# lazzati-astro/MCRaT

Hardware: AMD Instinct MI355X
Metric: photon-scatter-events/sec at 1e6 photons, 2D FLASH jet (higher is better)
Workload: dtype f64

## Files before the change

### include/mcrat_hip.h

```cpp
#ifndef MCRAT_HIP_H
#define MCRAT_HIP_H

#include <stddef.h>
#include <stdint.h>

#ifdef __cplusplus
extern "C" {
#endif
#if defined(__GNUC__)
#pragma GCC visibility push(default)
#endif

#define MCRAT_HIP_ABI_VERSION 1

#define MCRAT_HIP_OK        0
#define MCRAT_HIP_EINVAL   (-1)
#define MCRAT_HIP_ENODEV   (-2)
#define MCRAT_HIP_ENOMEM   (-3)
#define MCRAT_HIP_EHIP     (-4)
#define MCRAT_HIP_ESTATE   (-5)
#define MCRAT_HIP_EREFUSED (-6)

#define MCRAT_HIP_CARTESIAN        0
#define MCRAT_HIP_SPHERICAL        1
// ... 169 lines not shown
                            const mcrat_hip_outflow *outflow, mcrat_hip_ingest_result *result);

typedef struct mcrat_hip_hydro_columns {
    int num_elements;
    double *r0, *r1, *r2, *r0_size, *r1_size, *r2_size;
    double *v0, *v1, *v2;
    double *dens, *dens_lab, *pres, *temp, *gamma;
    double *r, *theta;
} mcrat_hip_hydro_columns;
int mcrat_hip_get_hydro(mcrat_hip_ctx *ctx, mcrat_hip_hydro_columns *out);

typedef struct mcrat_hip_output_columns {
    int count;
    double *p0, *p1, *p2, *p3;
    double *comv_p0, *comv_p1, *comv_p2, *comv_p3;
    double *r0, *r1, *r2;
    double *s0, *s1, *s2, *s3;
    double *num_scatt, *weight;
    char   *type;
} mcrat_hip_output_columns;
int mcrat_hip_get_output(mcrat_hip_ctx *ctx, mcrat_hip_output_columns *out);
int mcrat_hip_convert_comptonized(mcrat_hip_ctx *ctx, int *num_converted);
int mcrat_hip_get_photons_range(mcrat_hip_ctx *ctx, int first, int count, mcrat_hip_photon *records);

typedef struct mcrat_hip_outbox mcrat_hip_outbox;
int  mcrat_hip_outbox_create(mcrat_hip_ctx *ctx, mcrat_hip_outbox **box);
void mcrat_hip_outbox_destroy(mcrat_hip_outbox *box);
int  mcrat_hip_outbox_post(mcrat_hip_ctx *ctx, mcrat_hip_outbox *box, int want_records, int want_output);
int  mcrat_hip_outbox_wait(mcrat_hip_outbox *box, const mcrat_hip_photon **records, int *n_records, mcrat_hip_output_columns *cols);

typedef struct mcrat_hip_cyclosynch {
    int    b_field_calc;
    double epsilon_b;
    double rebin_e_perc, rebin_ang, rebin_ang_phi;
    int    scatt_frame_number, inj_frame_number;
} mcrat_hip_cyclosynch;
int mcrat_hip_set_hydro_extras(mcrat_hip_ctx *ctx, const double *dens, const double *B0, const double *B1, const double *B2);
int mcrat_hip_emit_cyclosynch_pool(mcrat_hip_ctx *ctx, const mcrat_hip_cyclosynch *cs, double r_inj, double ph_weight, int maximum_photons,
                                   double theta_min, double theta_max, double fps, uint64_t seed, int *num_emitted, double *ph_weight_adjusted,
                                   int *integrals_not_converged);
int mcrat_hip_rebin_cyclosynch(mcrat_hip_ctx *ctx, const mcrat_hip_cyclosynch *cs, int max_photons, int *empty_bins, int *num_cyclosynch_ph_emit,
                               int *scatt_cyclosynch_num_ph);
typedef struct mcrat_hip_cyclosynch_counts {
    int    num_cyclosynch_ph_emit, scatt_cyclosynch_num_ph, frame_abs_cnt;
    int    rebins;
    int    integrals_not_converged;
// ... 249 lines not shown
```

### mcrat_amd/csrc/device_types.hpp

```cpp
#pragma once
#include <stddef.h>
#include <stdint.h>

namespace mcrat {

constexpr double A_RAD = 7.56e-15;
constexpr double C_LIGHT = 2.99792458e10;
constexpr double PL_CONST = 6.6260755e-27;
constexpr double K_B = 1.380658e-16;
constexpr double M_P = 1.6726231e-24;
constexpr double THOM_X_SECT = 6.65246e-25;
constexpr double M_EL = 9.1093879e-28;

constexpr int GEOM_CARTESIAN = 0, GEOM_SPHERICAL = 1, GEOM_CYLINDRICAL = 2, GEOM_POLAR = 3;
constexpr int DIM_TWO = 0, DIM_TWO_POINT_FIVE = 1, DIM_THREE = 2;

constexpr unsigned FLAG_RECALC = 1u;
constexpr unsigned FLAG_MOVES = 2u;
constexpr unsigned FLAG_VALID = 4u;
constexpr unsigned FLAG_TAU_FRESH = 8u;

constexpr int TOPK = 4;
constexpr int MAX_SEG = 8;
constexpr int STEP_BLOCK = 256;
constexpr int STEP_QCAP = 1024;
#ifndef MCRAT_EVENT_BLOCK
#define MCRAT_EVENT_BLOCK 256
#endif
constexpr int SHORTLIST_CAP = MCRAT_EVENT_BLOCK;
constexpr int EVENT_BLOCK = MCRAT_EVENT_BLOCK;

struct PhotonDev {
    double *r0, *r1, *r2;
    double *p0, *p1, *p2, *p3;
    double *c0, *c1, *c2, *c3;
    double *s0, *s1, *s2, *s3;
    double *num_scatt;
    double *weight;
    double *tau;
    double *tts;
    double *u0, *u1, *u2;
    double *ntau;
    double *tau_next;
// ... 189 lines not shown
```

### mcrat_amd/csrc/engine.hip

```cpp
#include <hip/hip_runtime.h>
#include <algorithm>
#include <chrono>
#include <cmath>
#include <cstdio>
#include <cstdlib>
#include <cstring>
#include <mutex>
#include <new>
#include <string>
#include <vector>

#include "../../include/mcrat_hip.h"
#include "device_types.hpp"
#include "launch.hpp"
#include "observe_plan.hpp"
#include "sky_plan.hpp"
#include "sightline_plan.hpp"
#include "radfield_plan.hpp"
#include "comoving_plan.hpp"
#include "photon_cols.hpp"
#include "photon_plan.hpp"
#include "rng.hpp"

using namespace mcrat;
// ... 1734 lines not shown
    HIPCHK(c, hipMemcpyAsync(l->photons, c->aos_buf, bytes, hipMemcpyDeviceToHost, c->stream));
    HIPCHK(c, hipStreamSynchronize(c->stream));
    if (c->cfg.cyclosynchrotron_switch) {
        int nulls = 0;
        for (int i = 0; i < n; ++i) nulls += l->photons[i].type == 'N';
        l->num_null_photons = nulls;
        l->num_photons = n - nulls;
    }
    return MCRAT_HIP_OK;
}

extern "C" int mcrat_hip_get_photons_range(mcrat_hip_ctx *c, int first, int count, mcrat_hip_photon *records)
{
    if (!c || !records || first < 0 || count <= 0) return MCRAT_HIP_EINVAL;
    if (!c->have_photons) return MCRAT_HIP_ESTATE;
    if ((long long)first + count > c->ph.n) return MCRAT_HIP_EINVAL;
    int rc = flush_pending(c);
    if (rc) return rc;
    const size_t bytes = sizeof(mcrat_hip_photon) * (size_t)count;
    if ((rc = ensure_aos(c, bytes))) return rc;
    HIPCHK(c, hipMemsetAsync(c->aos_buf, 0, bytes, c->stream));
    HIPCHK(c, launch_soa_to_aos(c->ph, c->aos_buf, first, count, c->stream));
    HIPCHK(c, hipMemcpyAsync(records, c->aos_buf, bytes, hipMemcpyDeviceToHost, c->stream));
    HIPCHK(c, hipStreamSynchronize(c->stream));
    return MCRAT_HIP_OK;
}

extern "C" int mcrat_hip_convert_comptonized(mcrat_hip_ctx *c, int *num_converted)
{
    if (!c) return MCRAT_HIP_EINVAL;
    if (!c->have_photons) return MCRAT_HIP_ESTATE;
    int rc = ensure_aos(c, sizeof(unsigned));
    if (rc) return rc;
    unsigned n = 0;
    HIPCHK(c, hipMemsetAsync(c->aos_buf, 0, sizeof(unsigned), c->stream));
    HIPCHK(c, launch_convert_comptonized(c->ph, static_cast<unsigned *>(c->aos_buf), c->stream));
    HIPCHK(c, hipMemcpyAsync(&n, c->aos_buf, sizeof n, hipMemcpyDeviceToHost, c->stream));
    HIPCHK(c, hipStreamSynchronize(c->stream));
    if (num_converted) *num_converted = (int)n;
    return MCRAT_HIP_OK;
}

static size_t output_scan_ints(long long nblk) { return (size_t)nblk + 1 + grid_scan_scratch_ints(nblk); }
static int write_output(mcrat_hip_ctx *c, const OutputLayout &lay, void *base, long long nblk, unsigned long long total, OutputCols *oc)
{
    char *b = static_cast<char *>(base);
// ... 2505 lines not shown
```

### mcrat_amd/csrc/kernels.hip

```cpp
#include <hip/hip_runtime.h>
#include <limits.h>
#include <math.h>
#include <stdio.h>
#include <type_traits>
#include "device_types.hpp"
#include "launch.hpp"
#include "sc_exchange.hpp"
#include "physics.hpp"
#include "photon_cols.hpp"
#include "rng.hpp"
#include "cs_device.hpp"

#if !defined(MCRAT_TAU_TABLE_TU) || !defined(MCRAT_TU_DIMS)
#error "compile kernels.hip through kernels_d*.hip / kernels_table_d*.hip"
#endif
#define MCRAT_NS_CAT2(a, b) a##b
#define MCRAT_NS_CAT(a, b) MCRAT_NS_CAT2(a, b)
#if MCRAT_TAU_TABLE_TU
#define MCRAT_TU_NS MCRAT_NS_CAT(tau_table_d, MCRAT_TU_DIMS)
#else
#define MCRAT_TU_NS MCRAT_NS_CAT(tau_direct_d, MCRAT_TU_DIMS)
#endif

namespace mcrat {
// ... 204 lines not shown
        }
        if (queue == 1) bucket = phys::grid_bucket_of<DIMS>(hy.grid, a0, a1, a2);
        if (queue) return INFINITY;
        if (MC_DIAG(DIAG_SKIP_SAMPLE)) return 1e-3 + (double)i * 1e-12 + (double)(bits & 1) * 0.0 + ntau * 0.0;
        return sample_free_time(ntau, bits);
    }
    if (cell != -1) ph.idx(i) = -1;
    return 1e12 / C_LIGHT;
}

__device__ __forceinline__ double free_time_from_log(double ntau, double log_u) { return div_by_c(ntau * log_u); }

struct TableSite {
    uint64_t seed, pass;
    uint32_t stream, slot_base;
    int first;
    int mode;
    bool deferred;
    double norm, eps, theta;
    __device__ __forceinline__ TableSite(const RngKey &key, unsigned long long iter, int first_ = 0, int mode_ = 0)
        : seed(key.seed), pass(iter), stream(key.stream), slot_base(key.slot_base), first(first_), mode(mode_), deferred(false), norm(1), eps(0), theta(0) {}
};

template <int DIMS, int GEOM, bool LOGS = false, class PH>
__device__ __forceinline__ double slow_one(const PH &ph, const HydroDev &hy, int i, bool relocate, int bucket, bool count_it,
                                           uint64_t bits, int &relocated, int &not_found, TableSite &ts)
{
    const double r0 = ph.r0(i), r1 = ph.r1(i), r2 = ph.r2(i);
    const double p0 = ph.p0(i), p1 = ph.p1(i), p2 = ph.p2(i), p3 = ph.p3(i);
    const unsigned fl = ph.flags(i);
    int cell;
    bool need_tau = (fl & FLAG_RECALC) != 0;
    bool new_cell = false;
    double fa = 0, fb = 0, fc = 0, fw = 0, fnsig = 0, fgam = 1, fkf = 0.5;
    double a0 = 0, a1 = 0, a2 = 0;
    if (MC_DIAG(DIAG_SLOW_EMPTY)) { ph.tts(i) = 1e-3 + i * 1e-12; return 1e-3 + i * 1e-12; }
    if (MC_DIAG(DIAG_SLOW_NO_SEARCH)) relocate = false;
    if (relocate) {
        phys::hydro_coords<DIMS, GEOM>(r0, r1, r2, a0, a1, a2);
        FatCell hit;
        cell = phys::find_in_bucket<DIMS>(hy, bucket, a0, a1, a2, hit);
        ph.idx(i) = cell;
        if (cell != -1) {
            fa = hit.a; fb = hit.b; fc = hit.c; fw = hit.w; fnsig = hit.nsig; fgam = hit.gam; fkf = phys::kf_of_gamma(hit.gam);
            new_cell = true;
            need_tau = true;
            if (count_it) relocated += 1;
        } else {
            not_found += 1;
        }
    } else {
        cell = ph.idx(i);
        if (cell != -1) {
            const CellFluid f = hy.fluid[cell];
            fa = f.a; fb = f.b; fc = f.c; fw = f.w; fnsig = f.nsig;
        }
    }
    double t;
    if (MC_DIAG(DIAG_SLOW_NO_PHYSICS)) need_tau = false;
    if (cell != -1) {
        double ntau;
        if (need_tau) {
            double cphi, sphi;
            if (new_cell) phys::relocation_azimuth<DIMS, GEOM>(r0, r1, a0, cphi, sphi);
            else phys::cos_sin_of_atan2(r1, r0, cphi, sphi);
            double beta[3];
            phys::beta_from_record<DIMS>(fa, fb, fc, cphi, sphi, beta);
            double comv0 = 0;
            if (new_cell) {
                const double lab[4] = {p0, p1, p2, p3};
                double comv[4];
                phys::boost_with<true>(beta, fgam, fkf, lab, comv);
                ph.c0(i) = comv[0]; ph.c1(i) = comv[1]; ph.c2(i) = comv[2]; ph.c3(i) = comv[3];
                comv0 = comv[0];
            }
            double norm = 1.0;
            if constexpr (TABLE_MODE) {
                if (!new_cell) comv0 = ph.c0(i);
                if (ts.mode == 2) {
                    norm = ts.norm;
                } else if (phys::thermal_cross_section_lookup(hy, comv0, hy.temp[cell], norm, ts.eps, ts.theta)) {
                    if (ts.mode == 1) {
                        ts.deferred = true;
                        if (new_cell && count_it) relocated -= 1;
                        return 0.0;
                    }
                    norm = phys::table_fallback_lane(ts.eps, ts.theta, ts.seed, ts.pass, ts.slot_base + (uint32_t)(i - ts.first), ts.stream, hy.hot_fallback_calls);
                    atomicAdd(hy.table_fallbacks, 1);
                }
            }
            const double tau = phys::optical_depth_staged(beta, fw, fnsig, p1, p2, p3, norm);
            ntau = -phys::rcp_nr(tau);
            ph.tau(i) = tau;
            ph.ntau(i) = ntau;
            if (fl & FLAG_RECALC) ph.flags(i) = (unsigned char)(fl & ~(FLAG_RECALC | FLAG_TAU_FRESH));
        } else {
            ntau = ph.ntau(i);
        }
        t = LOGS ? free_time_from_log(ntau, __longlong_as_double((long long)bits)) : sample_free_time(ntau, bits);
    } else {
        t = 1e12 / C_LIGHT;
    }
    ph.tts(i) = t;
    return t;
}

struct LockstepProbe {
    const int *cached;
    bool force;
    bool *same;
};

template <int DIMS, int GEOM, int K, bool LOGS, bool COVERED, class PH>
__device__ __forceinline__ void relocate_lockstep_impl(const PH &ph, const HydroDev &hy, const int (&slot)[K], bool (&todo)[K],
                                                       const double (&r0)[K], const double (&r1)[K], const double (&a0)[K], const double (&a1)[K],
                                                       const double (&a2)[K], const int (&code)[K], const uint64_t (&bits)[K], const unsigned (&fl)[K],
                                                       bool count_it, double (&t)[K], int &relocated, const LockstepProbe *probe)
{
    static_assert(!TABLE_MODE, "DIRECT optical depths");
    const GridDev &g = hy.grid;
    double p0[K], p1[K], p2[K], p3[K];
    bool take[K];
    FatCell f[K];
    if constexpr (COVERED) {
        int cell[K];
#pragma unroll
        for (int k = 0; k < K; ++k) {
            take[k] = todo[k] && code[k] >= 0 && (code[k] & GRID_CODE_HINT_OK) != 0;
            cell[k] = phys::covered_cell<DIMS>(g, take[k] ? code[k] : 0);
            const int i = slot[k];
            p0[k] = ph.p0(i); p1[k] = ph.p1(i); p2[k] = ph.p2(i); p3[k] = ph.p3(i);
        }
#pragma unroll
        for (int k = 0; k < K; ++k) {
            take[k] = take[k] & (cell[k] >= 0);
            phys::fat_from_fluid(hy.fluid, take[k] ? cell[k] : 0, f[k]);
// ... 2 lines not shown
        BucketDir d[K];
#pragma unroll
        for (int k = 0; k < K; ++k) {
            take[k] = todo[k] && code[k] >= 0;
            d[k] = g.dir[take[k] ? (code[k] & GRID_CODE_BUCKET_MASK) : 0];
            const int i = slot[k];
            p0[k] = ph.p0(i); p1[k] = ph.p1(i); p2[k] = ph.p2(i); p3[k] = ph.p3(i);
        }
#pragma unroll
        for (int k = 0; k < K; ++k) {
            const unsigned hint = (d[k].hints >> (4 * ((code[k] >> GRID_CODE_OCT_SHIFT) & 7))) & 15u;
            take[k] = take[k] & (d[k].n > 0) & ((code[k] & GRID_CODE_HINT_OK) != 0) & (hint != GRID_NO_HINT);
            f[k] = g.cells[take[k] ? d[k].e0 + (int)hint : 0];
        }
    }
    double comv[K][4], tau[K], ntau[K];
#pragma unroll
    for (int k = 0; k < K; ++k) {
        if constexpr (!COVERED) take[k] = take[k] & phys::well_in_fat_cell<DIMS>(f[k], a0[k], a1[k], a2[k]);
        double cphi, sphi;
        phys::relocation_azimuth<DIMS, GEOM>(r0[k], r1[k], a0[k], cphi, sphi);
        double beta[3];
        phys::beta_from_record<DIMS>(f[k].a, f[k].b, f[k].c, cphi, sphi, beta);
        const double lab[4] = {p0[k], p1[k], p2[k], p3[k]};
        phys::boost_with<true>(beta, f[k].gam, phys::kf_of_gamma(f[k].gam), lab, comv[k]);
        tau[k] = phys::optical_depth_staged(beta, f[k].w, f[k].nsig, p1[k], p2[k], p3[k], 1.0);
        ntau[k] = -phys::rcp_nr(tau[k]);
        t[k] = LOGS ? free_time_from_log(ntau[k], __longlong_as_double((long long)bits[k])) : sample_free_time(ntau[k], bits[k]);
    }
#pragma unroll
    for (int k = 0; k < K; ++k)
        asm volatile("" : "+v"(comv[k][0]), "+v"(comv[k][1]), "+v"(comv[k][2]), "+v"(comv[k][3]), "+v"(tau[k]), "+v"(ntau[k]), "+v"(t[k]));
#pragma unroll
    for (int k = 0; k < K; ++k) {
        if (!take[k]) continue;
        if (probe) {
            probe->same[k] = !probe->force && f[k].cell == probe->cached[k];
            if (probe->same[k]) { todo[k] = false; continue; }
        }
        const int i = slot[k];
        ph.idx(i) = f[k].cell;
        ph.c0(i) = comv[k][0]; ph.c1(i) = comv[k][1]; ph.c2(i) = comv[k][2]; ph.c3(i) = comv[k][3];
        ph.tau(i) = tau[k];
        ph.ntau(i) = ntau[k];
        if (fl[k] & FLAG_RECALC) ph.flags(i) = (unsigned char)(fl[k] & ~(FLAG_RECALC | FLAG_TAU_FRESH));
        ph.tts(i) = t[k];
        if (count_it) relocated += 1;
        todo[k] = false;
    }
}
template <int DIMS, int GEOM, int K, bool LOGS = false, class PH>
__device__ __forceinline__ void relocate_lockstep(const PH &ph, const HydroDev &hy, const int (&slot)[K], bool (&todo)[K],
                                                  const double (&r0)[K], const double (&r1)[K], const double (&a0)[K], const double (&a1)[K],
                                                  const double (&a2)[K], const int (&code)[K], const uint64_t (&bits)[K], const unsigned (&fl)[K],
                                                  bool count_it, double (&t)[K], int &relocated, const LockstepProbe *probe = nullptr)
{
    if (hy.grid.cov_back) relocate_lockstep_impl<DIMS, GEOM, K, LOGS, true>(ph, hy, slot, todo, r0, r1, a0, a1, a2, code, bits, fl, count_it, t, relocated, probe);
    else relocate_lockstep_impl<DIMS, GEOM, K, LOGS, false>(ph, hy, slot, todo, r0, r1, a0, a1, a2, code, bits, fl, count_it, t, relocated, probe);
}

struct PairIn {
    double2 R0, R1, R2, U0, U1, U2, NTAU;
    int2 ID;
    uchar2 FL;
};

__device__ __forceinline__ PairIn load_pair(const PhotonDev &ph, int i0, bool need_u)
{
    PairIn in;
    in.R0 = *reinterpret_cast<const double2 *>(ph.r0 + i0);
    in.R1 = *reinterpret_cast<const double2 *>(ph.r1 + i0);
    in.R2 = *reinterpret_cast<const double2 *>(ph.r2 + i0);
    in.NTAU = *reinterpret_cast<const double2 *>(ph.ntau + i0);
    in.ID = *reinterpret_cast<const int2 *>(ph.idx + i0);
    in.FL = *reinterpret_cast<const uchar2 *>(ph.flags + i0);
    if (need_u) {
        in.U0 = *reinterpret_cast<const double2 *>(ph.u0 + i0);
        in.U1 = *reinterpret_cast<const double2 *>(ph.u1 + i0);
        in.U2 = *reinterpret_cast<const double2 *>(ph.u2 + i0);
    } else {
        in.U0 = in.U1 = in.U2 = make_double2(0, 0);
// ... 255 lines not shown
    ph.flags(i) = (unsigned char)(cand_flags | FLAG_RECALC | FLAG_TAU_FRESH);
}

struct CandCols {
    int idx;
    int cell;
    unsigned flags;
    double p[4], r[3], pc[4], u[3], s[4];
};
template <bool STOKES, class PH>
__device__ __forceinline__ void load_candidate(const PH &ph, int i, CandCols &c)
{
    c.idx = i;
    c.cell = ph.idx(i);
    c.p[0] = ph.p0(i); c.p[1] = ph.p1(i); c.p[2] = ph.p2(i); c.p[3] = ph.p3(i);
    c.r[0] = ph.r0(i); c.r[1] = ph.r1(i); c.r[2] = ph.r2(i);
    c.pc[0] = ph.c0(i); c.pc[1] = ph.c1(i); c.pc[2] = ph.c2(i); c.pc[3] = ph.c3(i);
    c.flags = ph.flags(i);
    c.u[0] = ph.u0(i); c.u[1] = ph.u1(i); c.u[2] = ph.u2(i);
    c.s[0] = 1; c.s[1] = 0; c.s[2] = 0; c.s[3] = 0;
    if constexpr (STOKES) { c.s[0] = ph.s0(i); c.s[1] = ph.s1(i); c.s[2] = ph.s2(i); c.s[3] = ph.s3(i); }
}

template <int DIMS, int GEOM, bool STOKES, bool WAVE = false, class PH, class SRC = KeyedSource>
__device__ __forceinline__ int try_candidate(const PH &ph, const HydroDev &hy, LoopState *st, const RngKey &key,
                                             unsigned long long iter, EventWalk &w, double scatt_time, int i, int slot_base, const SRC &src = SRC())
{
    const bool in_frame = scatt_time < w.dt_max;
    if (!(w.first && !in_frame)) w.last_idx = i;
    if (w.first) w.called = in_frame;
    w.first = false;
    if (!in_frame) {
        const double this_seg = w.dt_max - w.old_scatt_time;
        if (w.nseg < MAX_SEG) w.seg[w.nseg++] = this_seg;
        else w.seg[MAX_SEG - 1] += this_seg;
        w.dt = w.dt_max;
        return EV_DONE;
    }
    const double this_seg = scatt_time - w.old_scatt_time;
    if (w.nseg < MAX_SEG) w.seg[w.nseg++] = this_seg;
    else w.seg[MAX_SEG - 1] += this_seg;
    w.old_scatt_time = scatt_time;
    CandCols cc;
    load_candidate<STOKES>(ph, i, cc);
    const int cell = cc.cell;
    double p[4] = {cc.p[0], cc.p[1], cc.p[2], cc.p[3]};
    double r[3] = {cc.r[0], cc.r[1], cc.r[2]};
    double pc[4] = {cc.pc[0], cc.pc[1], cc.pc[2], cc.pc[3]};
    const unsigned cand_flags = cc.flags;
    const double u0 = cc.u[0], u1 = cc.u[1], u2 = cc.u[2];
    double s[4] = {cc.s[0], cc.s[1], cc.s[2], cc.s[3]};
    if (cell == -1) return EV_RUNNING;

    if (cand_flags & FLAG_MOVES) {
        for (int k = 0; k < w.nseg; ++k) {
            r[0] += u0 * w.seg[k];
            r[1] += u1 * w.seg[k];
            r[2] += u2 * w.seg[k];
        }
    }
    double fluid_temp, tau_new;
    if (!scatter_core<DIMS, GEOM, STOKES, WAVE, SRC>(hy, st, key, iter, (uint32_t)(i - slot_base) + key.slot_base, cell, r, p, pc, s, fluid_temp, tau_new, src)) {
        w.rej += 1;
        return EV_RUNNING;
    }
    commit_scatter<STOKES>(ph, i, p, pc, s, r, tau_new, cand_flags);
    st->frame_scatt_cnt += 1;
    st->last_scattered_temp = fluid_temp;
    w.skip = i;
    w.dt = scatt_time;
    MC_STAMP(st, 6);
    return EV_DONE;
}

template <int BLOCK>
struct EventSharedT {
    Cand w[BLOCK / 64][TOPK];
    Cand c[TOPK];
    Cand raw[BLOCK];
    Cand list[BLOCK];
    double wt[BLOCK / 64];
    int wi[BLOCK / 64];
    double seg[MAX_SEG];
    double last_t;
    int last_i;
    int status;
};
using EventShared = EventSharedT<EVENT_BLOCK>;

template <int DIMS, int GEOM, bool STOKES, int BLOCK, class PH, class SRC = KeyedSource>
__device__ __forceinline__ void event_block(const PH &ph, const HydroDev &hy, LoopState *st, const RngKey &key,
                                            EventSharedT<BLOCK> &sh, int n_raw, Cand gmin, int base, int n,
                                            unsigned long long iter, double dt_max, int last_idx, double t_est, const SRC &src = SRC())
{
    const int tid = threadIdx.x;
    int n_list = (n_raw > BLOCK) ? 0 : n_raw;
    if (tid < n_list) {
        const Cand me = sh.raw[tid];
        int rank = 0;
        for (int j = 0; j < n_list; ++j) rank += cand_less(sh.raw[j].t, sh.raw[j].idx, me.t, me.idx) ? 1 : 0;
        sh.list[rank] = me;
    }
    if (n_list == 0 && tid == 0) sh.list[0] = gmin;
    if (n_list > 64) __syncthreads();
    else __builtin_amdgcn_fence(__ATOMIC_ACQ_REL, "wavefront");
    if (n_list == 0 && gmin.idx != INT_MAX) n_list = 1;

    if (tid == 0) MC_STAMP(st, 1);
    EventWalk w;
    w.dt_max = dt_max;
    w.seg = sh.seg;
    w.old_scatt_time = 0; w.dt = 0; w.nseg = 0; w.skip = -1; w.rej = 0; w.first = true; w.called = false;
    w.last_idx = last_idx;
    long long rescans = 0;
    const double t_first = (n_list > 0) ? sh.list[0].t : INFINITY;

    const Cand *list = sh.list;
    const int max_rounds = n / TOPK + 3;
    for (int round = 0; round < max_rounds; ++round) {
        if (WAVE_WALK ? tid < 64 : tid == 0) {
#ifndef MCRAT_NO_WALK_PRIORITY
            __builtin_amdgcn_s_setprio(3);
#endif
            int status = EV_NEED_MORE;
            if (n_list == 0) {
                w.dt = (round == 0) ? w.dt_max : w.old_scatt_time;
                status = EV_DONE;
            }
            for (int c = 0; c < n_list && status == EV_NEED_MORE; ++c) {
                if (try_candidate<DIMS, GEOM, STOKES, WAVE_WALK>(ph, hy, st, key, iter, w, list[c].t, list[c].idx, base, src) == EV_DONE)
                    status = EV_DONE;
            }
            if (status == EV_NEED_MORE) {
                sh.last_t = list[n_list - 1].t;
                sh.last_i = list[n_list - 1].idx;
                rescans += 1;
            }
            sh.status = status;
#ifndef MCRAT_NO_WALK_PRIORITY
            __builtin_amdgcn_s_setprio(0);
#endif
        }
        __syncthreads();
        if (sh.status != EV_NEED_MORE) break;
        {
            const double lt = sh.last_t;
            const int li = sh.last_i;
            TopK more;
            more.init();
            for (int i = base + tid; i < base + n; i += BLOCK) {
                double t = ph.tts(i);
                if (t != t) t = INFINITY;
                if (cand_less(lt, li, t, i)) more.insert(t, i);
// ... 228 lines not shown
template <int BLOCK>
struct TapeLds {
    double u[BLOCK];
    int w[BLOCK / 64];
    long long pos, cursor;
};

#ifndef RANK_WAVES_PER_SIMD
#define RANK_WAVES_PER_SIMD 2
#endif
#ifndef RANK_NS_FUSED
#define RANK_NS_FUSED 2
#endif
#ifndef RANK_FUSE_DEN
#define RANK_FUSE_DEN 2
#endif

template <int DIMS, int GEOM, bool STOKES, bool RESIDENT, int RANK_BLOCK, bool FUSE, bool CSH = false, bool QUEUE = false, bool TAPE = false>
__global__ __launch_bounds__(RANK_BLOCK, RANK_WAVES_PER_SIMD) void rank_loop_kernel(PhotonDev gph, HydroDev hy_arg, LoopState *states, RngKey key,
                                                                std::conditional_t<TAPE, TapeLayout, RankLayout> lay, long long max_passes,
                                                                int lds_slots)
{
    constexpr int EVENT_BLOCK = RANK_BLOCK;
#ifndef RANK_NS_SPHERICAL
#define RANK_NS_SPHERICAL 4
#endif
    constexpr int RANK_NS_QUEUE = (GEOM == GEOM_SPHERICAL) ? RANK_NS_SPHERICAL : 4;
    constexpr int RANK_QCAP = 4 * RANK_BLOCK;
    extern __shared__ __align__(16) unsigned char s_dyn[];
    __shared__ LoopState st;
    __shared__ EventSharedT<RANK_BLOCK> sh;
    __shared__ int s_qn, s_sln, s_nrel, s_hook, s_len, s_item, s_ndefer;
    __shared__ int s_qb[RANK_QCAP];
    static_assert(sizeof(sh.list) >= sizeof(int) * RANK_QCAP, "queue fits into the sorted-list storage");
    int *const s_q = reinterpret_cast<int *>(sh.list);
    [[maybe_unused]] TapeLds<RANK_BLOCK> *tl = nullptr;
    if constexpr (TAPE) {
        __shared__ TapeLds<RANK_BLOCK> s_tape;
        tl = &s_tape;
    }
    int tid = threadIdx.x, lane = tid & 63;
    const bool queued = QUEUE ? lay.fq.n_frames > 0 : false;
    auto list_frame = [&](const int rank, const int item, const HydroDev &hy) __attribute__((always_inline)) {
    const int base = rank * lay.stride;
    int n = min(lay.stride, lay.n_total - base);
    RngKey rk = {key.seed, key.stream + (uint32_t)rank, 0u};
// ... 245 lines not shown
                    }
                    int qd[NS], code[NS];
                    bool settled[NS];
                    double tl[NS];
#pragma unroll
                    for (int k = 0; k < NS; ++k) { settled[k] = false; tl[k] = 0; qd[k] = 0; code[k] = -1; }
                    if constexpr (FUSED && !TABLE_MODE) {
                        bool cand[NS], same[NS], todo[NS];
                        bool any_todo = false;
#pragma unroll
                        for (int k = 0; k < NS; ++k) {
                            same[k] = false;
                            cand[k] = live[k] & ((fl[k] & FLAG_VALID) != 0) & dom[k] & (cell[k] != -1);
                            if (cand[k]) code[k] = phys::grid_bucket_of<DIMS>(hy.grid, a0[k], a1[k], a2[k]);
                            todo[k] = cand[k];
                            any_todo = any_todo || cand[k];
                        }
                        if (any_todo) {
                            int slot[NS];
#pragma unroll
                            for (int k = 0; k < NS; ++k) slot[k] = base + il[k];
                            const LockstepProbe probe = {cell, force, same};
                            double tt[NS];
                            relocate_lockstep<DIMS, GEOM, NS, true>(ph, hy, slot, todo, r0, r1, a0, a1, a2, code, bits, fl, !force, tt, relocated, &probe);
#pragma unroll
                            for (int k = 0; k < NS; ++k)
                                if (cand[k] && !todo[k] && !same[k]) { settled[k] = true; tl[k] = tt[k]; n_rel += 1; }
                        }
                        bool any = false;
#pragma unroll
                        for (int k = 0; k < NS; ++k) {
                            if (!cand[k]) continue;
                            bool stays = same[k];
                            if (todo[k]) {
                                stays = !force && phys::check_in_block<DIMS>(hy, cell[k], a0[k], a1[k], a2[k]);
                                if (!stays) { qd[k] = 1; n_rel += 1; }
                            }
                            if (stays && (fl[k] & FLAG_RECALC) && !(fl[k] & FLAG_TAU_FRESH)) qd[k] = 2;
                            any = any || (stays && qd[k] == 0);
                        }
                        if (any) {
#pragma unroll
                            for (int k = 0; k < NS; ++k) tf[k] = free_time_from_log(ntau[k], __longlong_as_double((long long)bits[k]));
                        }
                    } else {
#pragma unroll
                    for (int k = 0; k < NS; ++k) {
// ... 67 lines not shown
            TableSite ts(rk, iter, base, TABLE_MODE ? 1 : 0);
#pragma nounroll
            for (int round = 0; round < (TABLE_MODE ? 2 : 1); ++round) {
                if (round == 1) {
                    __syncthreads();
                    if (!s_ndefer) break;
                }
                const int e_step = round == 0 ? EVENT_BLOCK : EVENT_BLOCK / 64;
                for (int e = round == 0 ? tid : (tid >> 6); e < qn; e += e_step) {
                    const int q = s_q[e];
                    const int i = base + (q & ~(Q_RECALC_ONLY | Q_DEFERRED));
                    if constexpr (TABLE_MODE) {
                        if (round == 1) {
                            if (!(q & Q_DEFERRED)) continue;
                            const double norm = phys::table_fallback_wave(ph.tau(i), ph.ntau(i), ts.seed, ts.pass, ts.slot_base + (uint32_t)(i - base), ts.stream,
                                                                          hy.hot_fallback_calls);
                            if (lane != 0) continue;
                            atomicAdd(hy.table_fallbacks, 1);
                            ts.mode = 2;
                            ts.norm = norm;
                        }
                    }
                    const uint64_t qbits = (uint64_t)__double_as_longlong(ph.tts(i));
                    const double t = slow_one<DIMS, GEOM, true>(ph, hy, i, !(q & Q_RECALC_ONLY), s_qb[e], !force, qbits, relocated, not_found, ts);
                    if constexpr (TABLE_MODE) {
                        if (ts.deferred) {
                            ts.deferred = false;
                            ph.tau(i) = ts.eps;
                            ph.ntau(i) = ts.theta;
                            s_q[e] = q | Q_DEFERRED;
                            s_ndefer = 1;
                            continue;
                        }
                    }
                    best.offer(t, i);
                    if (t < t_cut) shortlist_lds(t, i);
                }
            }
        }
        if constexpr (TAPE) {
            if (taped) {
                __syncthreads();
                if (tid == 0) s_sln = 0;
                best.init();
                long long pos = tl->cursor;
                __syncthreads();
                for (int c0 = 0; c0 < n_pass; c0 += RANK_BLOCK) {
// ... 26 lines not shown
            if (lane == 63) {
                if (w_rel) atomicAdd(reinterpret_cast<unsigned long long *>(&st.n_relocated), (unsigned long long)w_rel);
                if (w_nf) atomicAdd(reinterpret_cast<unsigned long long *>(&st.not_found), (unsigned long long)w_nf);
            }
        }
        if (!force) RANK_TICK(11);
        __syncthreads();
        if (!force) RANK_TICK(12);
        prev_rel = s_nrel;
        MinCand g;
        g.init();
#pragma unroll
        for (int wv = 0; wv < EVENT_BLOCK / 64; ++wv) g.offer(sh.wt[wv], sh.wi[wv]);
        Cand gmin;
        gmin.t = g.t; gmin.idx = g.i; gmin.pad = 0;
        if (force) RANK_TICK(1); else RANK_TICK(13);
        const bool frame_goes_on = gmin.t < st.remaining_time;
        if constexpr (SHADOW) { if (frame_goes_on && tid >= 64) draw_logs(iter + 1, 64, RANK_BLOCK - 64); }
        (void)frame_goes_on;
        if constexpr (TAPE) {
            if (taped) event_block<DIMS, GEOM, STOKES, RANK_BLOCK>(ph, hy, &st, rk, sh, s_sln, gmin, base, n_pass, iter, st.remaining_time, st.last_scattered_index, st.t_est, tsrc);
            else event_block<DIMS, GEOM, STOKES, RANK_BLOCK>(ph, hy, &st, rk, sh, s_sln, gmin, base, n_pass, iter, st.remaining_time, st.last_scattered_index, st.t_est);
        } else {
            event_block<DIMS, GEOM, STOKES, RANK_BLOCK>(ph, hy, &st, rk, sh, s_sln, gmin, base, n_pass, iter, st.remaining_time, st.last_scattered_index, st.t_est);
        }
        if (tid == 0) {
            st.force_relocate = 0;
            s_hook = 0;
            if (lay.cs && st.photon_event_called) {
                const int sidx = st.last_scattered_index;
                const bool pool_photon = sidx >= 0 && gph.type[sidx] == 'p';
                const bool thousand = (st.frame_scatt_cnt % 1000 == 0) && st.frame_scatt_cnt != 0;
                if (pool_photon || thousand) {
                    if (CSH && lay.hook) {
                        s_hook = 1;
                    } else {
                        lay.cs[rank].halt = CS_HALT_HOOK;
                        lay.cs[rank].saved_done = st.done;
                        st.done = LOOP_CS_HALT;
                    }
                }
            }
        }
        __syncthreads();
        if constexpr (CSH) {
            if (s_hook) {
                apply_pending();
// ... 19 lines not shown
        }
        RANK_TICK(3);
#ifdef MCRAT_DIAG
        dg[5] += 1;
        if (!force) dg[14] += 1;
#endif
        if (st.done) break;
    }

    {
        apply_pending();
        __syncthreads();
        if constexpr (RESIDENT) {
            for (int il = tid; il < n; il += EVENT_BLOCK) {
                const int i = base + il;
                ph.template gcol<COL_R0>(i) = ph.r0(i); ph.template gcol<COL_R1>(i) = ph.r1(i); ph.template gcol<COL_R2>(i) = ph.r2(i);
                ph.template gcol<COL_NTAU>(i) = ph.ntau(i);
                if constexpr (FULL_HOT) {
                    ph.template gcol<COL_U0>(i) = ph.u0(i); ph.template gcol<COL_U1>(i) = ph.u1(i); ph.template gcol<COL_U2>(i) = ph.u2(i);
                    ph.g_idx_at(i) = ph.idx(i); ph.g_flags_at(i) = ph.flags(i);
                }
            }
        }
#ifdef MCRAT_DIAG
        __syncthreads();
        RANK_TICK(4);
        dg[2] = dg[9] + dg[10] + dg[11] + dg[12] + dg[13];
        if (tid == 0) for (int k = 0; k < 8; ++k) st.stamps[k] = (g_diag & 2048) ? (k < 6 ? dg[8 + k] : dg[k == 6 ? 5 : 14]) : dg[k];
        if (tid == 0 && dg_clock) {
            st.stamps[0] = dg_real0; st.stamps[1] = (long long)__builtin_amdgcn_s_memrealtime();
            st.stamps[2] = (long long)__builtin_amdgcn_s_memtime() - dg_tick0;
        }
#endif
        if (tid == 0) {
            st.nseg = 0; st.skip_idx = -1;
            if (st.last_scattered_index >= 0) st.last_scattered_index -= idx_shift;
            states[rank] = st;
            if (item >= 0) lay.fq.records[item].from_state(st);
            if constexpr (TAPE) lay.tapes[rank].cursor = tl->cursor;
        }
        if (item >= 0 && lay.fq.capture_delta != 0 && item / lay.n_ranks < lay.fq.n_frames - 1 && st.done == LOOP_DONE) {
            __syncthreads();
            copy_list_columns(gph.r0, gph.col_stride, gph.idx, gph.flags, gph.type, base, n, 0, lay.fq.capture_delta + (long long)(item / lay.n_ranks) * lay.fq.capture_stride, tid, RANK_BLOCK);
        }
    }
    };
// ... 702 lines not shown
```

### mcrat_amd/engine.py

```python
import ctypes as C
import os

import numpy as np

_HERE = os.path.dirname(os.path.abspath(__file__))
LIB_PATH = os.path.join(_HERE, "libmcrat_hip.so")

ABI_VERSION = 1
CARTESIAN, SPHERICAL, CYLINDRICAL, POLAR = 0, 1, 2, 3
TWO, TWO_POINT_FIVE, THREE = 0, 1, 2
TAU_DIRECT = 1
TAU_TABLE = 2

_dp = C.POINTER(C.c_double)
_ip = C.POINTER(C.c_int)

PHOTON_DTYPE = np.dtype(
    [("type", "S1"),
     ("p0", "f8"), ("p1", "f8"), ("p2", "f8"), ("p3", "f8"),
     ("comv_p0", "f8"), ("comv_p1", "f8"), ("comv_p2", "f8"), ("comv_p3", "f8"),
     ("r0", "f8"), ("r1", "f8"), ("r2", "f8"),
     ("s0", "f8"), ("s1", "f8"), ("s2", "f8"), ("s3", "f8"),
     ("num_scatt", "f8"),
     ("recalc_properties", "i4"),
# ... 219 lines not shown
    "mcrat_hip_init": (C.c_int, [C.POINTER(_ctx), C.POINTER(Config)]),
    "mcrat_hip_destroy": (None, [_ctx]),
    "mcrat_hip_version": (C.c_char_p, []),
    "mcrat_hip_strerror": (C.c_char_p, [C.c_int]),
    "mcrat_hip_last_error": (C.c_char_p, [_ctx]),
    "mcrat_hip_set_hydro": (C.c_int, [_ctx, C.POINTER(Hydro)]),
    "mcrat_hip_outflow_defaults": (None, [C.c_int, C.POINTER(Outflow)]),
    "mcrat_hip_ingest_flash": (C.c_int, [_ctx, C.POINTER(FlashBlocks), C.POINTER(Slab), C.POINTER(Outflow), C.POINTER(IngestResult)]),
    "mcrat_hip_ingest_pluto": (C.c_int, [_ctx, C.POINTER(PlutoGrid), C.POINTER(Slab), C.POINTER(Outflow), C.POINTER(IngestResult)]),
    "mcrat_hip_ingest_chombo": (C.c_int, [_ctx, C.POINTER(Chombo), C.POINTER(Slab), C.POINTER(Outflow), C.POINTER(IngestResult)]),
    "mcrat_hip_set_hydro_extras": (C.c_int, [_ctx, _dp, _dp, _dp, _dp]),
    "mcrat_hip_emit_cyclosynch_pool": (C.c_int, [_ctx, C.POINTER(Cyclosynch), C.c_double, C.c_double, C.c_int, C.c_double, C.c_double, C.c_double,
                                                 C.c_uint64, _ip, _dp, _ip]),
    "mcrat_hip_rebin_cyclosynch": (C.c_int, [_ctx, C.POINTER(Cyclosynch), C.c_int, _ip, _ip, _ip]),
    "mcrat_hip_scatter_frame_cyclosynch": (C.c_int, [_ctx, C.POINTER(Cyclosynch), _dp, C.c_double, C.c_uint64, C.c_double, C.c_double, C.c_int,
                                                     C.c_double, C.c_double, C.c_double, C.c_int, C.c_longlong, C.POINTER(FrameStats),
                                                     C.POINTER(CyclosynchCounts)]),
    "mcrat_hip_num_photon_slots": (C.c_int, [_ctx]),
    "mcrat_hip_absorb_cyclosynch": (C.c_int, [_ctx, C.POINTER(Cyclosynch), _ip, _ip, _dp]),
    "mcrat_hip_get_hydro": (C.c_int, [_ctx, C.POINTER(HydroColumns)]),
    "mcrat_hip_get_output": (C.c_int, [_ctx, C.POINTER(OutputColumns)]),
    "mcrat_hip_convert_comptonized": (C.c_int, [_ctx, _ip]),
    "mcrat_hip_get_photons_range": (C.c_int, [_ctx, C.c_int, C.c_int, C.c_void_p]),
    "mcrat_hip_inject_photons": (C.c_int, [_ctx, C.c_double, C.c_double, C.c_int, C.c_int, C.c_char, C.c_double, C.c_double, C.c_double,
                                           C.c_uint64, _ip, _dp]),
    "mcrat_hip_set_hot_cross_section": (C.c_int, [_ctx, _dp, C.c_int, C.c_int, C.c_double, C.c_double, C.c_double, C.c_double]),
    "mcrat_hip_table_fallback_calls": (C.c_int, [_ctx, C.c_int]),
    "mcrat_hip_pool_select_frame": (C.c_int, [_ctx, C.c_int]),
    "mcrat_hip_create_hot_cross_section": (C.c_int, [_ctx, _dp, C.c_int, C.c_int, C.c_double, C.c_double, C.c_double, C.c_double, C.c_longlong,
                                                     C.c_uint64]),
    "mcrat_hip_set_photons": (C.c_int, [_ctx, C.POINTER(PhotonList)]),
    "mcrat_hip_register_host": (C.c_int, [_ctx, C.c_void_p, C.c_size_t]),
    "mcrat_hip_unregister_host": (C.c_int, [_ctx, C.c_void_p]),
    "mcrat_hip_get_photons": (C.c_int, [_ctx, C.POINTER(PhotonList)]),
    "mcrat_hip_set_photons_soa": (C.c_int, [_ctx, C.POINTER(PhotonSoA)]),
    "mcrat_hip_get_photons_soa": (C.c_int, [_ctx, C.POINTER(PhotonSoA)]),
    "mcrat_hip_num_photon_slots": (C.c_int, [_ctx]),
    "mcrat_hip_pool_inject_photons": (C.c_int, [_ctx, C.c_double, C.POINTER(PoolInjectList)]),
    "mcrat_hip_pool_set_photons": (C.c_int, [_ctx, C.c_int, _ip, C.c_void_p]),
    "mcrat_hip_profile_totals": (C.c_int, [_ctx, C.POINTER(C.c_double), C.POINTER(C.c_longlong)]),
    "mcrat_hip_outbox_create": (C.c_int, [_ctx, C.POINTER(C.c_void_p)]),
    "mcrat_hip_outbox_destroy": (None, [C.c_void_p]),
    "mcrat_hip_outbox_post": (C.c_int, [_ctx, C.c_void_p, C.c_int, C.c_int]),
    "mcrat_hip_outbox_wait": (C.c_int, [C.c_void_p, C.POINTER(C.c_void_p), C.POINTER(C.c_int), C.c_void_p]),
    "mcrat_hip_bind_thread": (C.c_int, [_ctx]),
    "mcrat_hip_share_hydro": (C.c_int, [_ctx, _ctx]),
# ... 491 lines not shown
        self._check(self.lib.mcrat_hip_outbox_wait(box, C.byref(rec), C.byref(n), C.byref(o)), "outbox_wait")
        records = None
        if rec.value:
            records = np.frombuffer(C.string_at(rec, PHOTON_DTYPE.itemsize * n.value), dtype=PHOTON_DTYPE) if n.value else np.zeros(0, dtype=PHOTON_DTYPE)
        m = o.count
        cols = {f: np.ctypeslib.as_array(getattr(o, f), shape=(m,)).copy() if m else np.empty(0) for f in OUTPUT_COLUMNS}
        type_ptr = C.c_void_p.from_buffer(o, OutputColumns.type.offset).value
        cols["type"] = np.frombuffer(C.string_at(type_ptr, m), dtype="S1").copy() if m else np.empty(0, dtype="S1")
        return records, cols

    def outbox_destroy(self, box):
        self.lib.mcrat_hip_outbox_destroy(box)

    def convert_comptonized(self):
        n = C.c_int()
        self._check(self.lib.mcrat_hip_convert_comptonized(self.ctx, C.byref(n)), "convert_comptonized")
        return n.value

    def get_photons_range(self, first, count):
        a = np.zeros(count, dtype=PHOTON_DTYPE)
        self._check(self.lib.mcrat_hip_get_photons_range(self.ctx, int(first), int(count), a.ctypes.data), "get_photons_range")
        return a

    def set_photons_aos(self, aos, num_null=None):
        a = np.ascontiguousarray(aos, dtype=PHOTON_DTYPE)
        nulls = int(np.count_nonzero(a["type"] == b"N")) if num_null is None else int(num_null)
        l = PhotonList(a.ctypes.data, None, len(a) - nulls, nulls, len(a))
        self._check(self.lib.mcrat_hip_set_photons(self.ctx, C.byref(l)), "set_photons")
        self.n = len(a)

    def get_photons_aos(self, out=None):
        a = np.zeros(self.n, dtype=PHOTON_DTYPE) if out is None else out
        l = PhotonList(a.ctypes.data, None, self.n, 0, self.n)
        self._check(self.lib.mcrat_hip_get_photons(self.ctx, C.byref(l)), "get_photons")
        return a

    def register_host(self, array):
        self._check(self.lib.mcrat_hip_register_host(self.ctx, array.ctypes.data, array.nbytes), "register_host")

    def unregister_host(self, array):
        self._check(self.lib.mcrat_hip_unregister_host(self.ctx, array.ctypes.data), "unregister_host")

    def set_rng_tape(self, uniforms):
        if uniforms is None:
            self._check(self.lib.mcrat_hip_set_rng_tape(self.ctx, None, 0), "set_rng_tape")
            return
# ... 383 lines not shown
```

Before: 21.79 million.

## Defer comoving-frame boost on relocation until photon is scattered or pass ends

When a photon relocates to a new cell, the Lorentz boost to the comoving four-momentum is no longer computed right away. The code stores the azimuth and cell index in the comoving columns and sets a new lazy flag. The boost is computed on demand when the photon becomes a scatter candidate, and for all remaining flagged photons in a batched pass at the end of each rank pass. This avoids boosts for photons that relocate several times before scattering, but adds a full sweep over flags at pass end and overloads the comoving columns with temporary data. It also adds an API to read back the flag bytes.

```diff
diff --git a/include/mcrat_hip.h b/include/mcrat_hip.h
--- a/include/mcrat_hip.h
+++ b/include/mcrat_hip.h
@@ -215,6 +215,7 @@
 int mcrat_hip_get_output(mcrat_hip_ctx *ctx, mcrat_hip_output_columns *out);
 int mcrat_hip_convert_comptonized(mcrat_hip_ctx *ctx, int *num_converted);
 int mcrat_hip_get_photons_range(mcrat_hip_ctx *ctx, int first, int count, mcrat_hip_photon *records);
+int mcrat_hip_get_flag_bytes(mcrat_hip_ctx *ctx, int first, int count, unsigned char *flags);
 
 typedef struct mcrat_hip_outbox mcrat_hip_outbox;
 int  mcrat_hip_outbox_create(mcrat_hip_ctx *ctx, mcrat_hip_outbox **box);
diff --git a/mcrat_amd/csrc/device_types.hpp b/mcrat_amd/csrc/device_types.hpp
--- a/mcrat_amd/csrc/device_types.hpp
+++ b/mcrat_amd/csrc/device_types.hpp
@@ -19,6 +19,7 @@
 constexpr unsigned FLAG_MOVES = 2u;
 constexpr unsigned FLAG_VALID = 4u;
 constexpr unsigned FLAG_TAU_FRESH = 8u;
+constexpr unsigned FLAG_LAZY_COMV = 16u;
 
 constexpr int TOPK = 4;
 constexpr int MAX_SEG = 8;
diff --git a/mcrat_amd/csrc/engine.hip b/mcrat_amd/csrc/engine.hip
--- a/mcrat_amd/csrc/engine.hip
+++ b/mcrat_amd/csrc/engine.hip
@@ -1780,6 +1780,18 @@
     HIPCHK(c, hipMemsetAsync(c->aos_buf, 0, bytes, c->stream));
     HIPCHK(c, launch_soa_to_aos(c->ph, c->aos_buf, first, count, c->stream));
     HIPCHK(c, hipMemcpyAsync(records, c->aos_buf, bytes, hipMemcpyDeviceToHost, c->stream));
+    HIPCHK(c, hipStreamSynchronize(c->stream));
+    return MCRAT_HIP_OK;
+}
+
+extern "C" int mcrat_hip_get_flag_bytes(mcrat_hip_ctx *c, int first, int count, unsigned char *flags)
+{
+    if (!c || !flags || first < 0 || count <= 0) return MCRAT_HIP_EINVAL;
+    if (!c->have_photons) return MCRAT_HIP_ESTATE;
+    if ((long long)first + count > c->ph.n) return MCRAT_HIP_EINVAL;
+    int rc = flush_pending(c);
+    if (rc) return rc;
+    HIPCHK(c, hipMemcpyAsync(flags, c->ph.flags + first, (size_t)count, hipMemcpyDeviceToHost, c->stream));
     HIPCHK(c, hipStreamSynchronize(c->stream));
     return MCRAT_HIP_OK;
 }
diff --git a/mcrat_amd/csrc/kernels.hip b/mcrat_amd/csrc/kernels.hip
--- a/mcrat_amd/csrc/kernels.hip
+++ b/mcrat_amd/csrc/kernels.hip
@@ -250,7 +250,66 @@
         : seed(key.seed), pass(iter), stream(key.stream), slot_base(key.slot_base), first(first_), mode(mode_), deferred(false), norm(1), eps(0), theta(0) {}
 };
 
-template <int DIMS, int GEOM, bool LOGS = false, class PH>
+template <class PH>
+__device__ __forceinline__ void lazy_comv_record(const PH &ph, int i, double cphi, double sphi, int cell)
+{
+    ph.c0(i) = cphi; ph.c1(i) = sphi; ph.c2(i) = __longlong_as_double((long long)cell);
+}
+template <int DIMS>
+__device__ __forceinline__ void lazy_comv_boost(const CellFluid *fluid, int cell, double cphi, double sphi, const double lab[4], double comv[4])
+{
+    FatCell f;
+    phys::fat_from_fluid(fluid, cell, f);
+    double beta[3];
+    phys::beta_from_record<DIMS>(f.a, f.b, f.c, cphi, sphi, beta);
+    phys::boost_with<true>(beta, f.gam, phys::kf_of_gamma(f.gam), lab, comv);
+}
+template <int DIMS>
+__device__ __attribute__((noinline)) void materialise_lazy_comv(double *r0, unsigned col_stride, unsigned char *flags, const CellFluid *fluid, int base, int n,
+                                                                int tid, int block)
+{
+    constexpr int K = 4;
+    for (int il0 = tid; il0 < n; il0 += K * block) {
+        size_t i[K];
+        unsigned fl[K];
+        bool take[K];
+        int cell[K];
+        double cphi[K], sphi[K], lab[K][4], comv[K][4];
+        FatCell f[K];
+#pragma unroll
+        for (int k = 0; k < K; ++k) {
+            const int il = il0 + k * block;
+            take[k] = il < n;
+            i[k] = (size_t)base + (take[k] ? il : il0);
+            const double *const c = r0 + (size_t)COL_C0 * col_stride + i[k];
+            const double *const p = r0 + (size_t)COL_P0 * col_stride + i[k];
+            fl[k] = flags[i[k]];
+            cphi[k] = c[0]; sphi[k] = c[col_stride];
+            cell[k] = (int)__double_as_longlong(c[2 * (size_t)col_stride]);
+            lab[k][0] = p[0]; lab[k][1] = p[col_stride]; lab[k][2] = p[2 * (size_t)col_stride]; lab[k][3] = p[3 * (size_t)col_stride];
+        }
+#pragma unroll
+        for (int k = 0; k < K; ++k) {
+            take[k] = take[k] && (fl[k] & FLAG_LAZY_COMV) != 0;
+            phys::fat_from_fluid(fluid, take[k] ? cell[k] : 0, f[k]);
+        }
+#pragma unroll
+        for (int k = 0; k < K; ++k) {
+            double beta[3];
+            phys::beta_from_record<DIMS>(f[k].a, f[k].b, f[k].c, cphi[k], sphi[k], beta);
+            phys::boost_with<true>(beta, f[k].gam, phys::kf_of_gamma(f[k].gam), lab[k], comv[k]);
+        }
+#pragma unroll
+        for (int k = 0; k < K; ++k) {
+            if (!take[k]) continue;
+            double *const c = r0 + (size_t)COL_C0 * col_stride + i[k];
+            c[0] = comv[k][0]; c[col_stride] = comv[k][1]; c[2 * (size_t)col_stride] = comv[k][2]; c[3 * (size_t)col_stride] = comv[k][3];
+            flags[i[k]] = (unsigned char)(fl[k] & ~FLAG_LAZY_COMV);
+        }
+    }
+}
+
+template <int DIMS, int GEOM, bool LOGS = false, bool LAZY = false, class PH>
 __device__ __forceinline__ double slow_one(const PH &ph, const HydroDev &hy, int i, bool relocate, int bucket, bool count_it,
                                            uint64_t bits, int &relocated, int &not_found, TableSite &ts)
 {
@@ -295,7 +354,11 @@
             double beta[3];
             phys::beta_from_record<DIMS>(fa, fb, fc, cphi, sphi, beta);
             double comv0 = 0;
-            if (new_cell) {
+            unsigned keep = fl;
+            if (new_cell && LAZY) {
+                lazy_comv_record(ph, i, cphi, sphi, cell);
+                keep |= FLAG_LAZY_COMV;
+            } else if (new_cell) {
                 const double lab[4] = {p0, p1, p2, p3};
                 double comv[4];
                 phys::boost_with<true>(beta, fgam, fkf, lab, comv);
@@ -321,7 +384,12 @@
             ntau = -phys::rcp_nr(tau);
             ph.tau(i) = tau;
             ph.ntau(i) = ntau;
-            if (fl & FLAG_RECALC) ph.flags(i) = (unsigned char)(fl & ~(FLAG_RECALC | FLAG_TAU_FRESH));
+            if constexpr (LAZY) {
+                keep &= ~(FLAG_RECALC | FLAG_TAU_FRESH);
+                if (keep != fl) ph.flags(i) = (unsigned char)keep;
+            } else {
+                if (fl & FLAG_RECALC) ph.flags(i) = (unsigned char)(fl & ~(FLAG_RECALC | FLAG_TAU_FRESH));
+            }
         } else {
             ntau = ph.ntau(i);
         }
@@ -339,7 +407,7 @@
     bool *same;
 };
 
-template <int DIMS, int GEOM, int K, bool LOGS, bool COVERED, class PH>
+template <int DIMS, int GEOM, int K, bool LOGS, bool COVERED, bool LAZY, class PH>
 __device__ __forceinline__ void relocate_lockstep_impl(const PH &ph, const HydroDev &hy, const int (&slot)[K], bool (&todo)[K],
                                                        const double (&r0)[K], const double (&r1)[K], const double (&a0)[K], const double (&a1)[K],
                                                        const double (&a2)[K], const int (&code)[K], const uint64_t (&bits)[K], const unsigned (&fl)[K],
@@ -388,15 +456,21 @@
         phys::relocation_azimuth<DIMS, GEOM>(r0[k], r1[k], a0[k], cphi, sphi);
         double beta[3];
         phys::beta_from_record<DIMS>(f[k].a, f[k].b, f[k].c, cphi, sphi, beta);
-        const double lab[4] = {p0[k], p1[k], p2[k], p3[k]};
-        phys::boost_with<true>(beta, f[k].gam, phys::kf_of_gamma(f[k].gam), lab, comv[k]);
+        if constexpr (LAZY) {
+            comv[k][0] = cphi; comv[k][1] = sphi; comv[k][2] = 0; comv[k][3] = 0;
+        } else {
+            const double lab[4] = {p0[k], p1[k], p2[k], p3[k]};
+            phys::boost_with<true>(beta, f[k].gam, phys::kf_of_gamma(f[k].gam), lab, comv[k]);
+        }
         tau[k] = phys::optical_depth_staged(beta, f[k].w, f[k].nsig, p1[k], p2[k], p3[k], 1.0);
         ntau[k] = -phys::rcp_nr(tau[k]);
         t[k] = LOGS ? free_time_from_log(ntau[k], __longlong_as_double((long long)bits[k])) : sample_free_time(ntau[k], bits[k]);
     }
 #pragma unroll
-    for (int k = 0; k < K; ++k)
-        asm volatile("" : "+v"(comv[k][0]), "+v"(comv[k][1]), "+v"(comv[k][2]), "+v"(comv[k][3]), "+v"(tau[k]), "+v"(ntau[k]), "+v"(t[k]));
+    for (int k = 0; k < K; ++k) {
+        if constexpr (LAZY) asm volatile("" : "+v"(comv[k][0]), "+v"(comv[k][1]), "+v"(tau[k]), "+v"(ntau[k]), "+v"(t[k]));
+        else asm volatile("" : "+v"(comv[k][0]), "+v"(comv[k][1]), "+v"(comv[k][2]), "+v"(comv[k][3]), "+v"(tau[k]), "+v"(ntau[k]), "+v"(t[k]));
+    }
 #pragma unroll
     for (int k = 0; k < K; ++k) {
         if (!take[k]) continue;
@@ -406,23 +480,29 @@
         }
         const int i = slot[k];
         ph.idx(i) = f[k].cell;
-        ph.c0(i) = comv[k][0]; ph.c1(i) = comv[k][1]; ph.c2(i) = comv[k][2]; ph.c3(i) = comv[k][3];
+        if constexpr (LAZY) lazy_comv_record(ph, i, comv[k][0], comv[k][1], f[k].cell);
+        else { ph.c0(i) = comv[k][0]; ph.c1(i) = comv[k][1]; ph.c2(i) = comv[k][2]; ph.c3(i) = comv[k][3]; }
         ph.tau(i) = tau[k];
         ph.ntau(i) = ntau[k];
-        if (fl[k] & FLAG_RECALC) ph.flags(i) = (unsigned char)(fl[k] & ~(FLAG_RECALC | FLAG_TAU_FRESH));
+        if constexpr (LAZY) {
+            const unsigned keep = (fl[k] & ~(FLAG_RECALC | FLAG_TAU_FRESH)) | FLAG_LAZY_COMV;
+            if (keep != fl[k]) ph.flags(i) = (unsigned char)keep;
+        } else {
+            if (fl[k] & FLAG_RECALC) ph.flags(i) = (unsigned char)(fl[k] & ~(FLAG_RECALC | FLAG_TAU_FRESH));
+        }
         ph.tts(i) = t[k];
         if (count_it) relocated += 1;
         todo[k] = false;
     }
 }
-template <int DIMS, int GEOM, int K, bool LOGS = false, class PH>
+template <int DIMS, int GEOM, int K, bool LOGS = false, bool LAZY = false, class PH>
 __device__ __forceinline__ void relocate_lockstep(const PH &ph, const HydroDev &hy, const int (&slot)[K], bool (&todo)[K],
                                                   const double (&r0)[K], const double (&r1)[K], const double (&a0)[K], const double (&a1)[K],
                                                   const double (&a2)[K], const int (&code)[K], const uint64_t (&bits)[K], const unsigned (&fl)[K],
                                                   bool count_it, double (&t)[K], int &relocated, const LockstepProbe *probe = nullptr)
 {
-    if (hy.grid.cov_back) relocate_lockstep_impl<DIMS, GEOM, K, LOGS, true>(ph, hy, slot, todo, r0, r1, a0, a1, a2, code, bits, fl, count_it, t, relocated, probe);
-    else relocate_lockstep_impl<DIMS, GEOM, K, LOGS, false>(ph, hy, slot, todo, r0, r1, a0, a1, a2, code, bits, fl, count_it, t, relocated, probe);
+    if (hy.grid.cov_back) relocate_lockstep_impl<DIMS, GEOM, K, LOGS, true, LAZY>(ph, hy, slot, todo, r0, r1, a0, a1, a2, code, bits, fl, count_it, t, relocated, probe);
+    else relocate_lockstep_impl<DIMS, GEOM, K, LOGS, false, LAZY>(ph, hy, slot, todo, r0, r1, a0, a1, a2, code, bits, fl, count_it, t, relocated, probe);
 }
 
 struct PairIn {
@@ -724,7 +804,7 @@
     if constexpr (STOKES) { c.s[0] = ph.s0(i); c.s[1] = ph.s1(i); c.s[2] = ph.s2(i); c.s[3] = ph.s3(i); }
 }
 
-template <int DIMS, int GEOM, bool STOKES, bool WAVE = false, class PH, class SRC = KeyedSource>
+template <int DIMS, int GEOM, bool STOKES, bool WAVE = false, bool LAZY = false, class PH, class SRC = KeyedSource>
 __device__ __forceinline__ int try_candidate(const PH &ph, const HydroDev &hy, LoopState *st, const RngKey &key,
                                              unsigned long long iter, EventWalk &w, double scatt_time, int i, int slot_base, const SRC &src = SRC())
 {
@@ -749,7 +829,7 @@
     double p[4] = {cc.p[0], cc.p[1], cc.p[2], cc.p[3]};
     double r[3] = {cc.r[0], cc.r[1], cc.r[2]};
     double pc[4] = {cc.pc[0], cc.pc[1], cc.pc[2], cc.pc[3]};
-    const unsigned cand_flags = cc.flags;
+    unsigned cand_flags = cc.flags;
     const double u0 = cc.u[0], u1 = cc.u[1], u2 = cc.u[2];
     double s[4] = {cc.s[0], cc.s[1], cc.s[2], cc.s[3]};
     if (cell == -1) return EV_RUNNING;
@@ -759,6 +839,12 @@
             r[0] += u0 * w.seg[k];
             r[1] += u1 * w.seg[k];
             r[2] += u2 * w.seg[k];
+        }
+    }
+    if constexpr (LAZY) {
+        if (cand_flags & FLAG_LAZY_COMV) {
+            lazy_comv_boost<DIMS>(hy.fluid, cell, pc[0], pc[1], p, pc);
+            cand_flags &= ~FLAG_LAZY_COMV;
         }
     }
     double fluid_temp, tau_new;
@@ -790,7 +876,7 @@
 };
 using EventShared = EventSharedT<EVENT_BLOCK>;
 
-template <int DIMS, int GEOM, bool STOKES, int BLOCK, class PH, class SRC = KeyedSource>
+template <int DIMS, int GEOM, bool STOKES, int BLOCK, bool LAZY = false, class PH, class SRC = KeyedSource>
 __device__ __forceinline__ void event_block(const PH &ph, const HydroDev &hy, LoopState *st, const RngKey &key,
                                             EventSharedT<BLOCK> &sh, int n_raw, Cand gmin, int base, int n,
                                             unsigned long long iter, double dt_max, int last_idx, double t_est, const SRC &src = SRC())
@@ -830,7 +916,7 @@
                 status = EV_DONE;
             }
             for (int c = 0; c < n_list && status == EV_NEED_MORE; ++c) {
-                if (try_candidate<DIMS, GEOM, STOKES, WAVE_WALK>(ph, hy, st, key, iter, w, list[c].t, list[c].idx, base, src) == EV_DONE)
+                if (try_candidate<DIMS, GEOM, STOKES, WAVE_WALK, LAZY>(ph, hy, st, key, iter, w, list[c].t, list[c].idx, base, src) == EV_DONE)
                     status = EV_DONE;
             }
             if (status == EV_NEED_MORE) {
@@ -1105,6 +1191,7 @@
                                                                 int lds_slots)
 {
     constexpr int EVENT_BLOCK = RANK_BLOCK;
+    constexpr bool LAZY = !TABLE_MODE && !CSH && !TAPE;
 #ifndef RANK_NS_SPHERICAL
 #define RANK_NS_SPHERICAL 4
 #endif
@@ -1396,7 +1483,7 @@
                             for (int k = 0; k < NS; ++k) slot[k] = base + il[k];
                             const LockstepProbe probe = {cell, force, same};
                             double tt[NS];
-                            relocate_lockstep<DIMS, GEOM, NS, true>(ph, hy, slot, todo, r0, r1, a0, a1, a2, code, bits, fl, !force, tt, relocated, &probe);
+                            relocate_lockstep<DIMS, GEOM, NS, true, LAZY>(ph, hy, slot, todo, r0, r1, a0, a1, a2, code, bits, fl, !force, tt, relocated, &probe);
 #pragma unroll
                             for (int k = 0; k < NS; ++k)
                                 if (cand[k] && !todo[k] && !same[k]) { settled[k] = true; tl[k] = tt[k]; n_rel += 1; }
@@ -1510,7 +1597,7 @@
                         }
                     }
                     const uint64_t qbits = (uint64_t)__double_as_longlong(ph.tts(i));
-                    const double t = slow_one<DIMS, GEOM, true>(ph, hy, i, !(q & Q_RECALC_ONLY), s_qb[e], !force, qbits, relocated, not_found, ts);
+                    const double t = slow_one<DIMS, GEOM, true, LAZY>(ph, hy, i, !(q & Q_RECALC_ONLY), s_qb[e], !force, qbits, relocated, not_found, ts);
                     if constexpr (TABLE_MODE) {
                         if (ts.deferred) {
                             ts.deferred = false;
@@ -1583,7 +1670,7 @@
             if (taped) event_block<DIMS, GEOM, STOKES, RANK_BLOCK>(ph, hy, &st, rk, sh, s_sln, gmin, base, n_pass, iter, st.remaining_time, st.last_scattered_index, st.t_est, tsrc);
             else event_block<DIMS, GEOM, STOKES, RANK_BLOCK>(ph, hy, &st, rk, sh, s_sln, gmin, base, n_pass, iter, st.remaining_time, st.last_scattered_index, st.t_est);
         } else {
-            event_block<DIMS, GEOM, STOKES, RANK_BLOCK>(ph, hy, &st, rk, sh, s_sln, gmin, base, n_pass, iter, st.remaining_time, st.last_scattered_index, st.t_est);
+            event_block<DIMS, GEOM, STOKES, RANK_BLOCK, LAZY>(ph, hy, &st, rk, sh, s_sln, gmin, base, n_pass, iter, st.remaining_time, st.last_scattered_index, st.t_est);
         }
         if (tid == 0) {
             st.force_relocate = 0;
@@ -1649,6 +1736,7 @@
                 }
             }
         }
+        if constexpr (LAZY) materialise_lazy_comv<DIMS>(gph.r0, gph.col_stride, gph.flags, hy.fluid, base, n, tid, RANK_BLOCK);
 #ifdef MCRAT_DIAG
         __syncthreads();
         RANK_TICK(4);
diff --git a/mcrat_amd/engine.py b/mcrat_amd/engine.py
--- a/mcrat_amd/engine.py
+++ b/mcrat_amd/engine.py
@@ -265,6 +265,7 @@
     "mcrat_hip_get_output": (C.c_int, [_ctx, C.POINTER(OutputColumns)]),
     "mcrat_hip_convert_comptonized": (C.c_int, [_ctx, _ip]),
     "mcrat_hip_get_photons_range": (C.c_int, [_ctx, C.c_int, C.c_int, C.c_void_p]),
+    "mcrat_hip_get_flag_bytes": (C.c_int, [_ctx, C.c_int, C.c_int, C.c_void_p]),
     "mcrat_hip_inject_photons": (C.c_int, [_ctx, C.c_double, C.c_double, C.c_int, C.c_int, C.c_char, C.c_double, C.c_double, C.c_double,
                                            C.c_uint64, _ip, _dp]),
     "mcrat_hip_set_hot_cross_section": (C.c_int, [_ctx, _dp, C.c_int, C.c_int, C.c_double, C.c_double, C.c_double, C.c_double]),
@@ -802,6 +803,11 @@
         self._check(self.lib.mcrat_hip_get_photons_range(self.ctx, int(first), int(count), a.ctypes.data), "get_photons_range")
         return a
 
+    def get_flag_bytes(self, first, count):
+        a = np.zeros(int(count), dtype=np.uint8)
+        self._check(self.lib.mcrat_hip_get_flag_bytes(self.ctx, int(first), int(count), a.ctypes.data), "get_flag_bytes")
+        return a
+
     def set_photons_aos(self, aos, num_null=None):
         a = np.ascontiguousarray(aos, dtype=PHOTON_DTYPE)
         nulls = int(np.count_nonzero(a["type"] == b"N")) if num_null is None else int(num_null)
```

Result: slower. 21.56 million (-1.0%).
